# placeforyiming/DistanceTransform-DepthCompletion

Hardware: NVIDIA B200
Metric: DT+NN-fill frames/s @1216x352 (64-beam KITTI-shaped frames, batch 256 per GPU) (higher is better)
Workload: dtype u32 keys (integer chamfer) + f32 copy

## Files before the change

### distancetransform_depthcompletion_b200/csrc/dtfill.cu

```cuda
#include "dtfill.h"

#include <climits>
#include <cstdio>
#include <cstdlib>
#include <cstring>
#include <dlfcn.h>
#include <sched.h>

#include <atomic>
#include <condition_variable>
#include <functional>
#include <mutex>
#include <thread>
#include <string>
#include <vector>

#include "dtfill_kernels.cuh"

using namespace dtfill;

namespace {

thread_local std::string g_err;

// ... 214 lines not shown
                i = next_++;
                fn = fn_;
            }
            (*fn)(i);
            std::lock_guard<std::mutex> lk(mu_);
            if (++done_ == nparts_) cv_done_.notify_all();
        }
    }
    void loop() {
        for (;;) {
            {
                std::unique_lock<std::mutex> lk(mu_);
                cv_.wait(lk, [this] { return stop_ || next_ < nparts_; });
                if (stop_) return;
            }
            work();
        }
    }
    std::vector<std::thread> th_;
    std::mutex mu_;
    std::condition_variable cv_, cv_done_;
    bool stop_ = false;
    const std::function<void(size_t)>* fn_ = nullptr;
    size_t nparts_ = 0, next_ = 0, done_ = 0;
};

struct PinBuf {
    void* p = nullptr;
    size_t cap = 0;
};

struct Lane {
    static const int MAX_SUB = 16;
    Buf srcbits, wprefix, rowcell, rowsrc, rowval, counts, dlist, scratch, tasks, sky, skykeys;
    Buf ev_partial, ev_per_frame, ev_totals;
    bool ev_dirty = false;
    cudaStream_t sub[MAX_SUB] = {};
    cudaEvent_t fork_ev = nullptr, join_ev[MAX_SUB] = {};
    cudaStream_t side[MAX_SUB] = {};
    cudaEvent_t side_fork[MAX_SUB] = {}, side_join[MAX_SUB] = {};
    cudaStream_t pipe = nullptr;
    cudaStream_t pipe_front = nullptr;
    cudaEvent_t front_done = nullptr;
    cudaEvent_t done = nullptr;
    bool pending = false;
    int last_launches = 0;
    int last_B = 0;
};

struct dtfill_ctx {
    int device = 0;
    cudaStream_t own_stream = nullptr;
    cudaStream_t stream = nullptr;
    int sm_count = 148;
    static const int MAX_LANES = 4;
    Lane lanes[MAX_LANES];
    int ncalls = 0;
    int last_lane = 0;
    static const int STATUS_RING = 64;
    int* status_ring = nullptr;
    int* status_init = nullptr;
    bool slot_dirty[STATUS_RING] = {};
    cudaEvent_t slot_done[STATUS_RING] = {};
    int sticky_bad = INT_MAX;
    static const int STATUS_STRIDE = 64;
    int* status_dev = nullptr;
    bool slot_rearm[STATUS_RING] = {};
// ... 161 lines not shown
    if (is_src(ordered_to_float(lo))) return ordered_to_float(lo);
    while (hi - lo > 1) {
        const uint32_t mid = lo + (hi - lo) / 2;
        if (is_src(ordered_to_float(mid))) hi = mid; else lo = mid;
    }
    return ordered_to_float(hi);
}

int enqueue_range(dtfill_t* h, Lane* L, cudaStream_t s, cudaStream_t s_front, const Plan& plan, int b0, int nb, int Btot, const void* in, int H, int W,
                  float src_thr, float val_thr, float* out_depth, float* out_dt, int32_t* out_lbl, uint8_t* out_mask,
                  int32_t* out_counts, int scratch_units_per_frame, int sub_index, int* launches) {
    const int WW = (W + 31) / 32;
    const size_t rows0 = (size_t)b0 * H, npx0 = rows0 * W;
    const size_t rows = (size_t)nb * H;
    FrameParams fp;
    fp.B = nb; fp.H = H; fp.W = W; fp.WW = WW;
    fp.in_H = h->in_u16 ? h->in_H : H;
    fp.in_crop = h->in_u16 ? h->in_crop : 0;
    fp.src_thr = src_thr; fp.val_thr = val_thr;
    fp.src_cut = source_cut(src_thr);
    fp.init_dist = H + W + 8;
    fp.force_wide = plan.ppl == 0;
    fp.scratch_units_per_frame = scratch_units_per_frame;
    fp.wide_ppl = plan.ppl ? plan.ppl : 1;
    fp.narrow_ppl = (h->tiles2d && plan.ppl) ? plan.narrow : 0;
    fp.frame0 = b0;
    fp.sky_min = h->sky_min >= 0 ? h->sky_min : 8;
    fp.sky_split = (h->sky_split && !h->cur_pipelined && !h->profiling && h->tiles2d && plan.ppl && plan.narrow &&
                    h->narrow_main && fp.sky_min > 0 && W <= SKY_MAX_W && (long)Btot * H * W <= 28000000L) ? 1 : 0;
    fp.max_col_tiles = h->max_col_tiles;
    fp.mul_dist = 1u << (32 - DSH);
    fp.four = 4u;
    fp.one = 1u;
#ifdef DTFILL_TRACE
    fp.trace = h->trace_dev ? h->trace_dev + (size_t)(h->ncalls % dtfill_ctx::TRACE_CALLS) * 16 : nullptr;
#endif
    {
        int cap = h->band_cap;
        if (cap < 0) {
            const long beff = h->pipeline_depth > 1 ? (9L * Btot + 3) / 4 : Btot;
            const long per_frame = ((long)h->sm_count * 28 + beff - 1) / beff;
            if (per_frame <= 1) cap = 0;
            else {
                const long band_rows = (5L * H / 2) / per_frame;
                cap = (int)(2 * band_rows + 42);
                const int floor_cap = Btot <= 8 ? 80 : 96;
                if (cap < floor_cap) cap = floor_cap;
            }
        }
        fp.band_cap = plan.ppl ? cap : 0;
    }
    Workspace ws;
    ws.srcbits = (uint32_t*)L->srcbits.p + rows0 * WW;
    ws.wprefix = (uint16_t*)L->wprefix.p + rows0 * WW;
    ws.rowcell = (uint8_t*)L->rowcell.p + rows0 * WW;
    ws.rowsrc = (uint32_t*)L->rowsrc.p + rows0;
    ws.rowval = (uint32_t*)L->rowval.p + rows0;
    ws.counts = (int32_t*)L->counts.p + 2 * (size_t)b0;
    ws.dlist = (float*)L->dlist.p + npx0;
    ws.scratch = (uint32_t*)L->scratch.p + (size_t)b0 * scratch_units_per_frame * 32;
    ws.tasks = (Task*)L->tasks.p + (size_t)b0 * MAXT;
    ws.status = h->cur_status;
    ws.sky = (int*)L->sky.p + b0;
    ws.skykeys = (uint32_t*)L->skykeys.p + (size_t)b0 * 2 * W;
    float* olid = h->lidar_dev ? h->lidar_dev + npx0 : nullptr;
    float* od = out_depth + npx0;
    float* odt = out_dt ? out_dt + npx0 : nullptr;
    int32_t* ol = out_lbl ? out_lbl + npx0 : nullptr;
    uint8_t* om = out_mask ? out_mask + npx0 : nullptr;
    int32_t* oc = out_counts ? out_counts + 2 * (size_t)b0 : nullptr;

    if (h->profiling) CU(cudaEventRecord(h->ev[0], s));
    if (!(h->debug_skip & 1)) {
        const int k1_threads = 64;
        const int wpb = k1_threads / 32;
        long want = ((long)rows + wpb - 1) / wpb;
        int grid = (int)(want < 1 ? 1 : want);
        if (!h->in_u16) {
            const float* in_s = (const float*)in + npx0;
            if ((W & 15) == 0) k1_mask_rows_v16<float, true><<<grid, k1_threads, 0, s_front>>>(in_s, fp, ws, om, nullptr);
            else if ((W & 3) == 0) k1_mask_rows_v16<float, false><<<grid, k1_threads, 0, s_front>>>(in_s, fp, ws, om, nullptr);
            else k1_mask_rows<float><<<grid, k1_threads, 0, s_front>>>(in_s, fp, ws, om, nullptr);
        } else {
            const uint16_t* in_s = (const uint16_t*)in + (size_t)b0 * h->in_H * W;
            if ((W & 15) == 0) k1_mask_rows_v16<uint16_t, true><<<grid, k1_threads, 0, s_front>>>(in_s, fp, ws, om, olid);
            else if ((W & 7) == 0) k1_mask_rows_v16<uint16_t, false><<<grid, k1_threads, 0, s_front>>>(in_s, fp, ws, om, olid);
            else k1_mask_rows<uint16_t><<<grid, k1_threads, 0, s_front>>>(in_s, fp, ws, om, olid);
        }
        ++*launches;
        if (s_front != s) {
            CU(cudaEventRecord(L->front_done, s_front));
            CU(cudaStreamWaitEvent(s, L->front_done, 0));
        }
    }
    if (h->profiling) CU(cudaEventRecord(h->ev[1], s));
    if (!(h->debug_skip & 2)) {
        k1b_scan_compact<<<nb, K1B_THREADS, 0, s>>>(fp, ws, oc);
// ... 60 lines not shown
    if (h->profiling) CU(cudaEventRecord(h->ev[5], s));
    return 0;
}

int enqueue(dtfill_t* h, const void* in, int B, int H, int W, float src_thr, float val_thr, float* out_depth,
            float* out_dt, int32_t* out_lbl, uint8_t* out_mask, int32_t* out_counts, const HostIO* hio = nullptr,
            bool force_strict = false) {
    if (!h || !in || !out_depth) return fail(DTFILL_E_ARG, "dtfill_run: NULL handle, input or out_depth");
    if (B <= 0 || H <= 0 || W <= 0) return fail(DTFILL_E_ARG, "dtfill_run: B, H, W must be positive");
    if ((long)H + W >= 60000 || (long)H * W >= (1l << 31) || W > 28000)
        return fail(DTFILL_E_ARG, "dtfill_run: frame size not supported (H + W < 60000, W <= 28000)");
    CU(cudaSetDevice(h->device));
    const bool pipelined = h->pipeline_depth > 1 && !h->profiling && !hio && !force_strict;
    Lane* L = &h->lanes[pipelined ? (h->ncalls % h->pipeline_depth) : 0];
    h->cur_pipelined = pipelined;
    const Plan plan = make_plan(H, W);
    const int WW = (W + 31) / 32;
    const size_t rows = (size_t)B * H;
    const size_t npx = rows * W;

    int rc;
    if ((rc = ensure(h, L->srcbits, rows * WW * 4))) return rc;
    if ((rc = ensure(h, L->wprefix, rows * WW * 2))) return rc;
    if ((rc = ensure(h, L->rowcell, rows * WW))) return rc;
    if ((rc = ensure(h, L->rowsrc, rows * 4))) return rc;
    if ((rc = ensure(h, L->rowval, rows * 4))) return rc;
    if ((rc = ensure(h, L->counts, (size_t)B * 8))) return rc;
    if ((rc = ensure(h, L->dlist, npx * 4))) return rc;
    const int scratch_units_per_frame = plan.ppl ? 3 * H * plan.ppl : (int)(((size_t)H * W + 31) / 32);
    if ((rc = ensure(h, L->scratch, (size_t)B * scratch_units_per_frame * 128))) return rc;
    if ((rc = ensure(h, L->tasks, (size_t)B * MAXT * sizeof(Task)))) return rc;
    if ((rc = ensure(h, L->sky, (size_t)B * 4))) return rc;
    if ((rc = ensure(h, L->skykeys, (size_t)B * 2 * W * 4))) return rc;
    {
        const size_t smem = (size_t)3 * (W + 4) * sizeof(uint64_t);
        if (smem > 227 * 1024) return fail(DTFILL_E_ARG, "dtfill_run: frame too wide for the wide path");
        if (smem > 48 * 1024 && smem > h->wide_smem_configured) {
            CU(cudaFuncSetAttribute(k2_chamfer_wide, cudaFuncAttributeMaxDynamicSharedMemorySize, (int)smem));
            h->wide_smem_configured = smem;
        }
    }

    cudaStream_t s = h->stream, s_front = h->stream;
    if (pipelined) {
        CU(cudaEventRecord(h->pipe_fork, h->stream));
        s = L->pipe;
        if (h->prio_split) {
            s_front = L->pipe_front;
            CU(cudaStreamWaitEvent(s_front, h->pipe_fork, 0));
            if (L->pending) CU(cudaStreamWaitEvent(s_front, L->done, 0));
        } else {
            s_front = s;
            CU(cudaStreamWaitEvent(s, h->pipe_fork, 0));
        }
    } else {
        for (Lane& o : h->lanes)
            if (o.pending) { CU(cudaStreamWaitEvent(h->stream, o.done, 0)); o.pending = false; }
    }
    int launches = 0;
    const int slot = h->ncalls % dtfill_ctx::STATUS_RING;
    if (h->slot_dirty[slot]) {
        CU(cudaEventSynchronize(h->slot_done[slot]));
        if (h->status_ring[2 * slot] < h->sticky_bad) h->sticky_bad = h->status_ring[2 * slot];
        if (h->status_ring[2 * slot] != INT_MAX || h->status_ring[2 * slot + 1] != 0) h->slot_rearm[slot] = true;
        h->slot_dirty[slot] = false;
    }
// ... 214 lines not shown
        for (int i = 0; i < Lane::MAX_SUB; ++i) {
            CU(cudaStreamCreateWithFlags(&L.sub[i], cudaStreamNonBlocking));
            CU(cudaEventCreateWithFlags(&L.join_ev[i], cudaEventDisableTiming));
            CU(cudaStreamCreateWithPriority(&L.side[i], cudaStreamNonBlocking, prio_hi));
            CU(cudaEventCreateWithFlags(&L.side_fork[i], cudaEventDisableTiming));
            CU(cudaEventCreateWithFlags(&L.side_join[i], cudaEventDisableTiming));
        }
    }
    if (const char* e = getenv("DTFILL_PRIO_SPLIT")) h->prio_split = atoi(e) != 0;
    if (const char* e = getenv("DTFILL_TILES2D")) h->tiles2d = atoi(e) != 0;
    if (const char* e = getenv("DTFILL_SUBBATCHES")) h->nsub = atoi(e);
    if (const char* e = getenv("DTFILL_MAX_COL_TILES")) h->max_col_tiles = atoi(e);
    if (const char* e = getenv("DTFILL_SKY_MIN")) h->sky_min = atoi(e) < -1 ? -1 : atoi(e);
    if (const char* e = getenv("DTFILL_BAND_CAP")) h->band_cap = atoi(e);
    if (const char* e = getenv("DTFILL_NARROW_MAIN")) h->narrow_main = atoi(e) != 0;
    if (const char* e = getenv("DTFILL_SKY_SPLIT")) h->sky_split = atoi(e) != 0;
    if (const char* e = getenv("DTFILL_STAGE_THREADS")) h->stage_threads = atoi(e);
    if (const char* e = getenv("DTFILL_SPARSE_UPLOAD")) h->sparse_upload = atoi(e) != 0;
    if (const char* e = getenv("DTFILL_METRICS_EXACT")) h->metrics_exact = atoi(e) != 0;
    if (const char* e = getenv("DTFILL_PIPELINE_DEPTH")) {
        const int d = atoi(e);
        h->pipeline_depth = d < 1 ? 1 : (d > dtfill_ctx::MAX_LANES ? dtfill_ctx::MAX_LANES : d);
    }
    *out_handle = h;
    return 0;
}

void dtfill_destroy(dtfill_t* h) {
    if (!h) return;
    cudaSetDevice(h->device);
    cudaDeviceSynchronize();
    for (Lane& L : h->lanes) {
        Buf* lb[] = {&L.srcbits, &L.wprefix, &L.rowcell, &L.rowsrc, &L.rowval, &L.counts, &L.dlist,
                     &L.scratch, &L.tasks, &L.sky, &L.skykeys, &L.ev_partial, &L.ev_per_frame, &L.ev_totals};
        for (Buf* b : lb)
            if (b->p) cudaFree(b->p);
        if (L.fork_ev) cudaEventDestroy(L.fork_ev);
        if (L.done) cudaEventDestroy(L.done);
        if (L.pipe) cudaStreamDestroy(L.pipe);
        if (L.pipe_front) cudaStreamDestroy(L.pipe_front);
        if (L.front_done) cudaEventDestroy(L.front_done);
        for (int i = 0; i < Lane::MAX_SUB; ++i) {
            if (L.join_ev[i]) cudaEventDestroy(L.join_ev[i]);
            if (L.sub[i]) cudaStreamDestroy(L.sub[i]);
            if (L.side_fork[i]) cudaEventDestroy(L.side_fork[i]);
            if (L.side_join[i]) cudaEventDestroy(L.side_join[i]);
            if (L.side[i]) cudaStreamDestroy(L.side[i]);
        }
    }
    Buf* bufs[] = {&h->in_dev, &h->depth_dev, &h->dt_dev, &h->lbl_dev, &h->mask_dev, &h->counts_out_dev, &h->lidar_out_dev,
                   &h->gt_dev, &h->partial, &h->per_frame, &h->sums, &h->edt_rows, &h->edt_stack, &h->sparse_dev,
                   &h->mx_terms, &h->mx_counts, &h->mx_leaf_start, &h->mx_leaf_sum};
    for (Buf* b : bufs)
        if (b->p) cudaFree(b->p);
    for (void* q : h->retired) cudaFree(q);
    if (h->counts_host) cudaFreeHost(h->counts_host);
    delete h->pool_in;
    delete h->pool_out;
    for (PinBuf* b : {&h->pin_in, &h->pin_depth, &h->pin_dt, &h->pin_lbl, &h->pin_mask, &h->pin_lidar, &h->pin_sparse})
        if (b->p) cudaFreeHost(b->p);
    if (h->status_ring) cudaFreeHost(h->status_ring);
    if (h->status_dev) cudaFree(h->status_dev);
    if (h->status_stream) cudaStreamDestroy(h->status_stream);
    if (h->status_fork) cudaEventDestroy(h->status_fork);
    for (auto& e : h->slot_done)
        if (e) cudaEventDestroy(e);
    for (auto& e : h->ev)
// ... 738 lines not shown
```

### distancetransform_depthcompletion_b200/csrc/dtfill_common.cuh

```cuda
#pragma once
#include <cuda_runtime.h>
#include <stdint.h>

namespace dtfill {


constexpr int DSH = 21;
constexpr int OSH = 17;
constexpr uint32_t LMASK = (1u << OSH) - 1u;
constexpr uint32_t ORDCLR = ~(15u << OSH);
constexpr uint32_t MAX_FAST_LABEL = LMASK;
constexpr float UNREACHED_DT = 65533.0f;

__host__ __device__ constexpr uint32_t KC(int cost, int order) {
    return (uint32_t(cost) << DSH) | (uint32_t(order) << OSH);
}

enum TaskKind : int { TASK_CHAMFER = 0, TASK_NOSRC = 1, TASK_WIDE = 2, TASK_SKIP = 3, TASK_NARROW = 4 };

struct __align__(16) Task {
    int frame;
    int lo, hi;
    int r0, r1;
    int kind;
    int scratch_off;
    int fstart;
    int clo;
    int c0, c1;
    int sky;
};

constexpr int MAXT = 32;
constexpr int CELL_H = 4;
constexpr int CELL_W = 8;
constexpr int SKY_MAX_W = 1216;
constexpr int MAX_CELLS = 15360;

struct FrameParams {
    int B, H, W, WW;
    int in_H, in_crop;
    float src_thr, val_thr;
    float src_cut;
    int init_dist;
    int force_wide;
    int band_cap;
    int scratch_units_per_frame;
    int wide_ppl;
    int narrow_ppl;
    int max_col_tiles;
    int sky_min;
    int sky_split;
    int frame0;
    uint32_t mul_dist;
    uint32_t four;
    uint32_t one;
#ifdef DTFILL_TRACE
    unsigned long long* trace;
#endif
};

struct Workspace {
    uint32_t* srcbits;
    uint16_t* wprefix;
    uint8_t* rowcell;
    uint32_t* rowsrc;
    uint32_t* rowval;
    int32_t* counts;
    float* dlist;
    uint32_t* scratch;
    Task* tasks;
    int* sky;
    uint32_t* skykeys;
    int* status;
};

__device__ __forceinline__ float ld_stream(const float* p) {
    float v;
    asm volatile("ld.global.nc.L1::no_allocate.f32 %0, [%1];" : "=f"(v) : "l"(p));
    return v;
}
__device__ __forceinline__ void st_stream_u32(void* p, uint32_t v) {
    asm volatile("st.global.cs.u32 [%0], %1;" ::"l"(p), "r"(v));
}
__device__ __forceinline__ void st_stream_v4(void* p, uint32_t a, uint32_t b, uint32_t c, uint32_t d) {
    asm volatile("st.global.cs.v4.u32 [%0], {%1, %2, %3, %4};" ::"l"(p), "r"(a), "r"(b), "r"(c), "r"(d));
}
__device__ __forceinline__ float4 ld_stream_v4(const float* p) {
    float4 v;
    asm volatile("ld.global.nc.v4.f32 {%0, %1, %2, %3}, [%4];"
                 : "=f"(v.x), "=f"(v.y), "=f"(v.z), "=f"(v.w) : "l"(p));
    return v;
}
__device__ __forceinline__ uint4 ld_stream_v4u(const void* p) {
    uint4 v;
    asm volatile("ld.global.nc.v4.u32 {%0, %1, %2, %3}, [%4];" : "=r"(v.x), "=r"(v.y), "=r"(v.z), "=r"(v.w) : "l"(p));
    return v;
}
__device__ __forceinline__ float u16_depth(uint32_t v16) { return __uint_as_float(0x47000000u | v16) - 32768.0f; }
__device__ __forceinline__ float load_px_stream(const float* p) { return ld_stream(p); }
__device__ __forceinline__ float load_px_stream(const uint16_t* p) { return u16_depth(__ldg(p)); }

template <typename T> struct In16;
template <> struct In16<float> {
    float4 q[4];
    __device__ __forceinline__ void load(const float* p, int col, int W) {
// ... 80 lines not shown
```

### distancetransform_depthcompletion_b200/csrc/dtfill_k1b_plan.cuh

```cuda
#pragma once
#include "dtfill_common.cuh"

namespace dtfill {

constexpr int K1B_THREADS = 512;

__device__ __forceinline__ uint32_t block_exclusive_scan(uint32_t v, uint32_t* smem , uint32_t& total)
{
    constexpr int NW = K1B_THREADS / 32;
    const int lane = threadIdx.x & 31, wid = threadIdx.x >> 5;
    uint32_t inc = v;
#pragma unroll
    for (int d = 1; d < 32; d <<= 1) {
        const uint32_t o = __shfl_up_sync(0xffffffffu, inc, d);
        if (lane >= d) inc += o;
    }
    if (lane == 31) smem[wid] = inc;
    __syncthreads();
    if (threadIdx.x == 0) {
        uint32_t run = 0;
        for (int i = 0; i < NW; ++i) { const uint32_t t = smem[i]; smem[i] = run; run += t; }
        smem[NW] = run;
    }
    __syncthreads();
// ... 200 lines not shown
#pragma unroll
                for (int t = 0; t < 2; ++t) {
                    const uint32_t cin = __shfl_down_sync(0xffffffffu, e[t], 1);
                    d[t] = lane == 31 ? 120000u : cin;
                    mx[t] = 0;
#pragma unroll
                    for (int k = 7; k >= 0; --k)
                        if (k < chunk) { d[t] = min(d[t] + CELL_W, v[t][k]); if (xa + k < nw) mx[t] = max(mx[t], d[t]); }
                }
#pragma unroll
                for (int s_ = 16; s_ > 0; s_ >>= 1) {
#pragma unroll
                    for (int t = 0; t < 2; ++t) mx[t] = max(mx[t], __shfl_xor_sync(0xffffffffu, mx[t], s_));
                }
#pragma unroll
                for (int t = 0; t < 2; ++t) {
                    const int cy = cy0 + 8 * t;
                    if (lane == 0 && cy < nh) cellU[cy] = (int)min(mx[t], 60000u) + (CELL_H - 1) + (CELL_W - 1);
                }
            }
        } else {
            for (int cy = c0row + pw * 32 + lane; cy < nh; cy += 256) {
                uint32_t d = 60000;
                for (int cx = 0; cx < nw; ++cx) { d = min(d + CELL_W, (uint32_t)cellD[cy * nw + cx]); cellD[cy * nw + cx] = (uint16_t)min(d, 60000u); }
                d = 60000;
                uint32_t mx = 0;
                for (int cx = nw - 1; cx >= 0; --cx) { d = min(d + CELL_W, (uint32_t)cellD[cy * nw + cx]); mx = max(mx, min(d, 60000u)); }
                cellU[cy] = (int)mx + (CELL_H - 1) + (CELL_W - 1);
            }
        }
        planner_sync();
    }
    dbg_mark(4);

    if (ptid == 0) {
        ws.counts[2 * b] = (int)nsrc;
        ws.counts[2 * b + 1] = (int)nval;
        if (out_counts) { out_counts[2 * b] = (int)nsrc; out_counts[2 * b + 1] = (int)nval; }
        if (nval == 0 || nsrc > nval) atomicMin(&ws.status[0], b + fp.frame0);
        if (kind == TASK_WIDE) atomicAdd(&ws.status[1], 1);

        int nt = 0;
        Task* t = st;
        int* cost = scost;
        auto blank = [&](int knd) {
            Task q;
            q.frame = b; q.lo = 0; q.hi = H; q.r0 = 0; q.r1 = H; q.kind = knd; q.scratch_off = 0; q.fstart = 0;
            q.clo = 0; q.c0 = 0; q.c1 = W; q.sky = -2;
            return q;
        };
        int S = S0;
        if (plan) {
            const int nwid = fp.narrow_ppl * 32;
            int cy = S / CELL_H, scr = 0;
            bool ok = true;
            while (cy < nh && ok) {
                const int r0 = cy * CELL_H;
                int lo = 1 << 30, hi = 0, prev = 0, end = cy, best_lo = 0, best_hi = 0, umax = 0, best_u = 0;
                const bool base_band = fp.sky_split && S > 0 && r0 == S;
                for (int c = cy; c < nh; ++c) {
                    lo = min(lo, c * CELL_H - cellU[c]);
                    hi = max(hi, min(H, (c + 1) * CELL_H) + cellU[c]);
                    umax = max(umax, cellU[c]);
                    const int L = max(S, lo), Hh = min(H, hi);
                    const int cst = (Hh - L) + (Hh - r0);
                    const bool take = c == cy || (!base_band && (nt >= MAXT - 4 || cst <= fp.band_cap || cst - prev <= CELL_H ||
// ... 90 lines not shown
```

### distancetransform_depthcompletion_b200/csrc/dtfill_k2_chamfer.cuh

```cuda
#pragma once
#include "dtfill_common.cuh"

namespace dtfill {

template <int PPL>
struct Row {
    uint32_t v[PPL];
    uint32_t l1, l2;
    uint32_t r0, r1;
};

template <int PPL>
__device__ __forceinline__ uint32_t at(const Row<PPL>& r, int idx) {
    return idx == -2 ? r.l2 : idx == -1 ? r.l1 : idx == PPL ? r.r0 : idx == PPL + 1 ? r.r1 : r.v[idx < 0 ? 0 : (idx >= PPL ? PPL - 1 : idx)];
}

template <int PPL>
__device__ __forceinline__ void fill_row(Row<PPL>& r, uint32_t k) {
#pragma unroll
    for (int i = 0; i < PPL; ++i) r.v[i] = k;
    r.l1 = r.l2 = r.r0 = r.r1 = k;
}

template <int PPL>
// ... 57 lines not shown
}
__device__ __forceinline__ void st_scratch_v4_hint(void* p, uint32_t a, uint32_t b, uint32_t c, uint32_t d, uint64_t pol) {
    asm volatile("st.global.L2::cache_hint.v4.u32 [%0], {%1, %2, %3, %4}, %5;" ::"l"(p), "r"(a), "r"(b), "r"(c), "r"(d), "l"(pol) : "memory");
}
__device__ __forceinline__ void cp_async16_hint(uint32_t smem_addr, const void* gptr, uint64_t pol) {
    asm volatile("cp.async.cg.shared.global.L2::cache_hint [%0], [%1], 16, %2;" ::"r"(smem_addr), "l"(gptr), "l"(pol) : "memory");
}
__device__ __forceinline__ void l2_discard_128(const void* p) {
    asm volatile("discard.global.L2 [%0], 128;" ::"l"(p) : "memory");
}
__device__ __forceinline__ void mbar_init(uint32_t mbar, uint32_t count) {
    asm volatile("mbarrier.init.shared::cta.b64 [%0], %1;" ::"r"(mbar), "r"(count) : "memory");
    asm volatile("fence.mbarrier_init.release.cluster;" ::: "memory");
}
__device__ __forceinline__ void bulk_row_to_smem(uint32_t smem_dst, const void* gsrc, uint32_t bytes, uint32_t mbar) {
    asm volatile("mbarrier.arrive.expect_tx.shared::cta.b64 _, [%0], %1;" ::"r"(mbar), "r"(bytes) : "memory");
    asm volatile("cp.async.bulk.shared::cluster.global.mbarrier::complete_tx::bytes [%0], [%1], %2, [%3];"
                 ::"r"(smem_dst), "l"(gsrc), "r"(bytes), "r"(mbar) : "memory");
}
__device__ __forceinline__ void mbar_wait(uint32_t mbar, uint32_t parity) {
    uint32_t done = 0;
    while (!done)
        asm volatile("{\n\t.reg .pred p;\n\tmbarrier.try_wait.parity.shared::cta.b64 p, [%1], %2;\n\tselp.u32 %0, 1, 0, p;\n\t}"
                     : "=r"(done) : "r"(mbar), "r"(parity) : "memory");
}
__device__ __forceinline__ void cp_async_commit() { asm volatile("cp.async.commit_group;" ::: "memory"); }
template <int N>
__device__ __forceinline__ void cp_async_wait() { asm volatile("cp.async.wait_group %0;" ::"n"(N) : "memory"); }

__device__ __forceinline__ float key_dist_f32(uint32_t key, uint32_t mul_dist) {
    uint32_t t;
    asm("mad.hi.u32 %0, %1, %2, %3;" : "=r"(t) : "r"(key), "r"(mul_dist), "r"(0x4B000000u));
    return __uint_as_float(t) - 8388608.0f;
}

struct RowBits {
    uint32_t a, b, c, pre, base;
};

template <int PPL>
__device__ __forceinline__ RowBits fetch_row_bits(const uint32_t* __restrict__ bits_f, const uint16_t* __restrict__ pre_f,
                                                  const uint32_t* __restrict__ rowbase, int WW, int x0, int y)
{
    RowBits r;
    const int w = x0 >> 5;
    const uint32_t* br = bits_f + (long)y * WW;
    r.a = w < WW ? br[w] : 0u;
    r.b = w + 1 < WW ? br[w + 1] : 0u;
    r.c = (PPL > 33 && w + 2 < WW) ? br[w + 2] : 0u;
    r.pre = w < WW ? (uint32_t)pre_f[(long)y * WW + w] : 0u;
    r.base = rowbase[y];
    return r;
}

template <int PPL>
struct LaneBits { typedef uint64_t type; };
template <> struct LaneBits<10> { typedef uint32_t type; };
template <> struct LaneBits<20> { typedef uint32_t type; };

template <int PPL>
__device__ __forceinline__ void decode_row_bits(const RowBits& r, int x0, typename LaneBits<PPL>::type& bits,
                                                uint32_t& rank)
{
    const int sh = x0 & 31;
    if (sizeof(typename LaneBits<PPL>::type) == 4) {
        bits = __funnelshift_r(r.a, r.b, sh) & ((1u << (PPL & 31)) - 1u);
    } else {
        uint64_t lo = ((uint64_t)r.b << 32) | r.a;
        lo >>= sh;
        if (PPL > 33 && sh) lo |= (uint64_t)r.c << (64 - sh);
        bits = (typename LaneBits<PPL>::type)(lo & ((PPL >= 64) ? ~0ull : ((1ull << PPL) - 1ull)));
    }
    rank = r.base + r.pre + __popc(r.a & ((1u << sh) - 1u)) + 1u;
}


#ifndef DTFILL_STENCIL
#define DTFILL_STENCIL 1
#endif
#ifndef DTFILL_SPLITSCAN
#define DTFILL_SPLITSCAN 1
#endif
#ifndef DTFILL_FAKE_SCRATCH_DIV
#define DTFILL_FAKE_SCRATCH_DIV 1
#endif
#ifndef DTFILL_L2POLICY
#define DTFILL_L2POLICY 0
#endif
#ifndef DTFILL_K2_TMA
#define DTFILL_K2_TMA 1
#endif
#ifndef DTFILL_FLUSH_LATE
#define DTFILL_FLUSH_LATE 0
#endif
#ifndef DTFILL_K2_SMEMROW
#define DTFILL_K2_SMEMROW 0
#endif
#ifndef DTFILL_K2_WARPS
#define DTFILL_K2_WARPS (DTFILL_K2_SMEMROW ? 28 : 20)
#endif

template <int PPL>
__device__ __forceinline__ void load_row_smem(Row<PPL>& r, const uint32_t* row, int lane, uint32_t init_key) {
    const uint4* p = reinterpret_cast<const uint4*>(row + lane * PPL);
#pragma unroll
    for (int j = 0; j < PPL / 4; ++j) {
        const uint4 q = p[j];
        r.v[4 * j] = q.x; r.v[4 * j + 1] = q.y; r.v[4 * j + 2] = q.z; r.v[4 * j + 3] = q.w;
    }
    const uint32_t a = row[lane == 0 ? 0 : lane * PPL - 1], c = row[lane == 31 ? 0 : lane * PPL + PPL];
    r.l1 = lane == 0 ? init_key : a;
    r.r0 = lane == 31 ? init_key : c;
    r.l2 = r.r1 = init_key;
}
template <int PPL>
__device__ __forceinline__ void store_row_smem(uint32_t* row, const Row<PPL>& r, int lane) {
    uint4* p = reinterpret_cast<uint4*>(row + lane * PPL);
#pragma unroll
    for (int j = 0; j < PPL / 4; ++j) p[j] = make_uint4(r.v[4 * j], r.v[4 * j + 1], r.v[4 * j + 2], r.v[4 * j + 3]);
}

template <int PPL>
__device__ __forceinline__ uint32_t stencil_fwd(const Row<PPL>& A , const Row<PPL>& Bq , int i, uint32_t one)
{
    const uint32_t b0 = at(Bq, i - 1), b1 = at(Bq, i + 1);
    const uint32_t a0 = at(A, i - 2), a1 = at(A, i - 1), a2 = at(A, i), a3 = at(A, i + 1), a4 = at(A, i + 2);
#if DTFILL_STENCIL == 0
    uint32_t m = b0 * one + KC(3, 0);
    m = __viaddmin_u32(b1, KC(3, 2), m);
    m = __viaddmin_u32(a0, KC(3, 4), m);
    m = __viaddmin_u32(a1, KC(2, 6), m);
    m = __viaddmin_u32(a2, KC(1, 8), m);
// ... 65 lines not shown
    __shared__ __align__(16) uint2 fwdbuf[16 * PPL];
#if DTFILL_K2_TMA
    __shared__ __align__(8) uint64_t fwdbar;
#endif

    const Task task = ws.tasks[blockIdx.x];
    if (task.kind != my_kind && !(task.kind == TASK_NOSRC && my_kind == TASK_CHAMFER)) return;
    DTFILL_TRACE_SCOPE(fp, 2);
    const int lane = threadIdx.x;
    const int H = fp.H, W = fp.W, WW = fp.WW;
    const int b = task.frame;
    const long fpx = (long)b * H * W;

    if (task.kind == TASK_NOSRC) {
        const int nval = ws.counts[2 * b + 1];
        const float last = ws.dlist[fpx + (nval > 0 ? nval - 1 : 0)];
        for (long i = (long)task.r0 * W + lane; i < (long)task.r1 * W; i += 32) {
            out_depth[fpx + i] = last;
            if (out_dt) out_dt[fpx + i] = UNREACHED_DT;
            if (WANT_LBL) out_lbl[fpx + i] = 0;
        }
        return;
    }

    const int x0 = task.clo + lane * PPL;
    const int xl = lane * PPL;
    const uint32_t init_key = (uint32_t)fp.init_dist << DSH;
    const uint32_t clamp_dist = 2047u - PPL - 1u;
    const uint32_t* bits_f = ws.srcbits + (long)b * H * WW;
    const uint16_t* pre_f = ws.wprefix + (long)b * H * WW;
    const uint32_t* rowbase = ws.rowsrc + (long)b * H;
    constexpr int VW = (PPL % 4 == 0) ? 4 : 2;
    uint2* scr = reinterpret_cast<uint2*>(ws.scratch) + (long)task.scratch_off * 16;

#if DTFILL_L2POLICY
    const uint64_t pol_keep = l2_policy_evict_last(), pol_drop = l2_policy_evict_first();
#endif
    Row<PPL> ra, rb;
    fill_row(ra, init_key);
    fill_row(rb, init_key);

    RowBits nextbits = fetch_row_bits<PPL>(bits_f, pre_f, rowbase, WW, x0, task.fstart);
    auto fwd_step = [&](const Row<PPL>& A , Row<PPL>& Bq , int y) {
        typename LaneBits<PPL>::type bits; uint32_t rank;
        decode_row_bits<PPL>(nextbits, x0, bits, rank);
        nextbits = fetch_row_bits<PPL>(bits_f, pre_f, rowbase, WW, x0, min(y + 1, task.hi - 1));
        if (lane < 2 && y + 4 < task.hi) {
            asm volatile("prefetch.global.L2 [%0];" ::"l"(bits_f + (long)(y + 4) * WW + (x0 >> 5) + lane * 32));
            asm volatile("prefetch.global.L2 [%0];" ::"l"(pre_f + (long)(y + 4) * WW + (x0 >> 5) + lane * 32));
        }
        uint32_t c[PPL];
#pragma unroll
        for (int i = 0; i < PPL; ++i) c[i] = stencil_fwd<PPL>(A, Bq, i, fp.one);
        if (__any_sync(0xffffffffu, bits != 0)) {
#pragma unroll
            for (int i = 0; i < PPL; ++i) {
                const bool s = (bits & ((typename LaneBits<PPL>::type)1 << i)) != 0;
                c[i] = s ? rank : c[i];
                rank += s ? 1u : 0u;
            }
        }
#if DTFILL_SPLITSCAN
        constexpr int HF = PPL / 2;
        uint32_t u = c[0] & ORDCLR, u2 = c[HF] & ORDCLR;
        c[0] = u; c[HF] = u2;
#pragma unroll
        for (int i = 1; i < PPL - HF; ++i) {
            if (i < HF) { u = __viaddmin_u32(u, KC(1, 14), c[i]) & ORDCLR; c[i] = u; }
            u2 = __viaddmin_u32(u2, KC(1, 14), c[HF + i]) & ORDCLR; c[HF + i] = u2;
        }
        const uint32_t e = __viaddmin_u32(u | (1u << OSH), uint32_t(PPL - HF) << DSH, u2) & ORDCLR;
        const uint32_t cin = lane_carry<PPL, +1>(e, lane, clamp_dist);
        const uint32_t cin2 = __viaddmin_u32(cin, uint32_t(HF) << DSH, u) | (1u << OSH);
#pragma unroll
        for (int i = 0; i < PPL; ++i) {
            uint32_t t = i < HF ? __viaddmin_u32(cin, uint32_t(i + 1) << DSH, c[i])
                                : __viaddmin_u32(cin2, uint32_t(i - HF + 1) << DSH, c[i]);
            if (PAD && x0 + i >= W) t = init_key;
            Bq.v[i] = t;
        }
#else
        uint32_t u = c[0] & ORDCLR;
        c[0] = u;
#pragma unroll
        for (int i = 1; i < PPL; ++i) {
            u = __viaddmin_u32(u, KC(1, 14), c[i]) & ORDCLR;
            c[i] = u;
        }
        const uint32_t cin = lane_carry<PPL, +1>(u, lane, clamp_dist);
#pragma unroll
        for (int i = 0; i < PPL; ++i) {
            uint32_t t = __viaddmin_u32(cin, uint32_t(i + 1) << DSH, c[i]);
            if (PAD && x0 + i >= W) t = init_key;
            Bq.v[i] = t;
        }
#endif
        refresh_halo(Bq, lane, init_key);
        if (y >= task.r0) {
            char* dst = reinterpret_cast<char*>(scr) + (long)(y - task.lo) * (128 * PPL) + lane * (4 * VW);
#pragma unroll
            for (int j = 0; j < PPL / VW / DTFILL_FAKE_SCRATCH_DIV; ++j) {
#if DTFILL_L2POLICY
                if (VW == 4) st_scratch_v4_hint(dst + j * 512, Bq.v[4 * j], Bq.v[4 * j + 1], Bq.v[4 * j + 2], Bq.v[4 * j + 3], pol_keep);
#else
                if (VW == 4) st_scratch_v4(dst + j * 512, Bq.v[4 * j], Bq.v[4 * j + 1], Bq.v[4 * j + 2], Bq.v[4 * j + 3]);
#endif
                else st_scratch_v2(dst + j * 256, Bq.v[2 * j], Bq.v[2 * j + 1]);
            }
        }
    };

    if (SB) {
        store_row_smem<PPL>(stage_ring, ra, lane);
        store_row_smem<PPL>(stage_ring + 32 * PPL, ra, lane);
        __syncwarp();
#pragma unroll 1
        for (int y = task.fstart; y < task.hi; ++y) {
            uint32_t* slot = stage_ring + (y & 1) * (32 * PPL);
            load_row_smem<PPL>(rb, slot, lane, init_key);
            fwd_step(ra, rb, y);
            __syncwarp();
            store_row_smem<PPL>(slot, rb, lane);
            ra = rb;
        }
        __syncwarp();
    } else {
#pragma unroll 1
    for (int y = task.fstart; y < task.hi; ++y) {
        fwd_step(ra, rb, y);
        const Row<PPL> t = ra; ra = rb; rb = t;
    }
// ... 13 lines not shown
    uint32_t okmask = 0;
#pragma unroll
    for (int j = 0; j < NJ; ++j) {
        const int lc = (j * 32 + lane) * 4, col = task.clo + lc;
        if (lc < 32 * PPL && col >= task.c0 && col < task.c1) okmask |= 1u << j;
    }
    const long colbase = fpx + task.clo + lane * 4;
    const uint4* sread0 = reinterpret_cast<const uint4*>(&stage[lane * 4]);
    uint2* swrite0 = reinterpret_cast<uint2*>(&stage[xl]);
    const uint32_t fwdbuf_lane = (uint32_t)__cvta_generic_to_shared(fwdbuf) + lane * (4 * VW);

#if DTFILL_K2_TMA
    constexpr bool TMA_ROWS = (VW == 4) && DTFILL_FAKE_SCRATCH_DIV == 1;
#else
    constexpr bool TMA_ROWS = false;
#endif
#if DTFILL_K2_TMA
    const uint32_t fwdbar_a = (uint32_t)__cvta_generic_to_shared(&fwdbar);
    const uint32_t fwdbuf_a = (uint32_t)__cvta_generic_to_shared(fwdbuf);
    if (TMA_ROWS) {
        if (lane == 0) mbar_init(fwdbar_a, 1);
        asm volatile("fence.proxy.async;" ::: "memory");
        __syncwarp();
    }
    uint32_t fwd_phase = 0;
    bool fwd_inflight = false;
#endif
    auto issue_fwd_row = [&](int y) {
        const bool have = y >= task.fstart && y >= task.lo;
#if DTFILL_K2_TMA
        if (TMA_ROWS) {
            fwd_inflight = have;
            if (have && lane == 0)
                bulk_row_to_smem(fwdbuf_a, reinterpret_cast<const char*>(scr) + (long)(y - task.lo) * (128 * PPL), 128 * PPL, fwdbar_a);
            return;
        }
#endif
        if (have) {
            const char* src = reinterpret_cast<const char*>(scr) + (long)(y - task.lo) * (128 * PPL) + lane * (4 * VW);
#pragma unroll
            for (int j = 0; j < PPL / VW / DTFILL_FAKE_SCRATCH_DIV; ++j) {
#if DTFILL_L2POLICY
                if (VW == 4) cp_async16_hint(fwdbuf_lane + j * 512, src + j * 512, pol_drop);
#else
                if (VW == 4) cp_async16_l2only(fwdbuf_lane + j * 512, src + j * 512);
#endif
                else cp_async8(fwdbuf_lane + j * 256, src + j * 256);
            }
        }
        cp_async_commit();
    };
    auto wait_fwd_row = [&]() {
#if DTFILL_K2_TMA
        if (TMA_ROWS) {
            if (fwd_inflight) { mbar_wait(fwdbar_a, fwd_phase); fwd_phase ^= 1u; }
            return;
        }
#endif
        cp_async_wait<0>();
    };
    uint32_t g[NJ * 4];
    auto flush_depth_row = [&](int y) {
        float* pd = out_depth + colbase + (long)y * W;
#pragma unroll
        for (int j = 0; j < NJ; ++j)
            if ((okmask >> j) & 1u) st_stream_v4(pd + j * 128, g[4 * j], g[4 * j + 1], g[4 * j + 2], g[4 * j + 3]);
    };

    issue_fwd_row(task.hi - 1);

    auto bwd_step = [&](const Row<PPL>& A , Row<PPL>& Bq , int y) {
        if (lane < PPL / DTFILL_FAKE_SCRATCH_DIV && y - 3 >= task.fstart)
            asm volatile("prefetch.global.L2 [%0];" ::"l"(reinterpret_cast<const char*>(scr) +
                                                          (long)(y - 3 - task.lo) * (128 * PPL) + lane * 128));
#if DTFILL_FLUSH_LATE == 0
        if (VEC && y + 1 >= task.r0 && y + 1 < task.r1) flush_depth_row(y + 1);
#endif
        wait_fwd_row();
#if DTFILL_L2POLICY >= 2
        if (VW == 4 && lane < PPL && y >= task.fstart && y >= task.lo)
            l2_discard_128(reinterpret_cast<const char*>(scr) + (long)(y - task.lo) * (128 * PPL) + lane * 128);
#endif
        uint32_t c[PPL];
        if (y >= task.fstart) {
#pragma unroll
            for (int j = 0; j < PPL / VW; ++j) {
                if (DTFILL_FAKE_SCRATCH_DIV > 1 && j >= PPL / VW / DTFILL_FAKE_SCRATCH_DIV) {
                    for (int e = 0; e < VW; ++e) c[VW * j + e] = init_key;
                } else if (VW == 4) {
                    const uint4 f = reinterpret_cast<const uint4*>(fwdbuf)[j * 32 + lane];
                    c[4 * j] = f.x; c[4 * j + 1] = f.y; c[4 * j + 2] = f.z; c[4 * j + 3] = f.w;
                } else {
                    const uint2 f = fwdbuf[j * 32 + lane];
                    c[2 * j] = f.x; c[2 * j + 1] = f.y;
                }
            }
        } else {
#pragma unroll
            for (int i = 0; i < PPL; ++i) c[i] = init_key;
        }
#pragma unroll
        for (int i = 0; i < PPL; ++i) c[i] = stencil_bwd<PPL>(c[i], A, Bq, i, fp.one) & ORDCLR;
#if DTFILL_K2_TMA
        if (TMA_ROWS) __syncwarp();
#endif
        issue_fwd_row(y - 1);
#if DTFILL_FLUSH_LATE == 1
        if (VEC && y + 1 >= task.r0 && y + 1 < task.r1) flush_depth_row(y + 1);
#endif
#if DTFILL_SPLITSCAN
        constexpr int HF = PPL / 2;
        uint32_t u = c[PPL - 1], u2 = c[HF - 1];
#pragma unroll
        for (int i = 1; i < PPL - HF; ++i) {
            u = __viaddmin_u32(u, KC(1, 1), c[PPL - 1 - i]) & ORDCLR; c[PPL - 1 - i] = u;
            if (i < HF) { u2 = __viaddmin_u32(u2, KC(1, 1), c[HF - 1 - i]) & ORDCLR; c[HF - 1 - i] = u2; }
        }
// ... 113 lines not shown
```

Before: 614,300.

## Compress forward-pass scratch rows to 16-bit keys when cell bounds allow

New measurement: 585,400, median of 6. -4.7%, worse.

```diff
diff --git a/distancetransform_depthcompletion_b200/csrc/dtfill.cu b/distancetransform_depthcompletion_b200/csrc/dtfill.cu
--- a/distancetransform_depthcompletion_b200/csrc/dtfill.cu
+++ b/distancetransform_depthcompletion_b200/csrc/dtfill.cu
@@ -270,7 +270,7 @@
 
 struct Lane {
     static const int MAX_SUB = 16;
-    Buf srcbits, wprefix, rowcell, rowsrc, rowval, counts, dlist, scratch, tasks, sky, skykeys;
+    Buf srcbits, wprefix, rowcell, rowsrc, rowval, counts, dlist, scratch, tasks, sky, skykeys, cellu;
     Buf ev_partial, ev_per_frame, ev_totals;
     bool ev_dirty = false;
     cudaStream_t sub[MAX_SUB] = {};
@@ -498,6 +498,13 @@
     fp.mul_dist = 1u << (32 - DSH);
     fp.four = 4u;
     fp.one = 1u;
+    fp.m16 = 1u << 16;
+    for (int f = 0; f < 2; ++f) {
+        const uint32_t db = 4 + f, ob = 16 - db;
+        fp.f16[f].m32 = 1u << (32 - ob); fp.f16[f].mo = 1u << ob; fp.f16[f].m16o = 1u << (16 + ob);
+        fp.f16[f].sat2 = ((1u << db) - 1u) * 0x10001u;
+        fp.f16[f].md = 1u << db; fp.f16[f].kd = (1u << DSH) - (1u << ob);
+    }
 #ifdef DTFILL_TRACE
     fp.trace = h->trace_dev ? h->trace_dev + (size_t)(h->ncalls % dtfill_ctx::TRACE_CALLS) * 16 : nullptr;
 #endif
@@ -529,6 +536,7 @@
     ws.status = h->cur_status;
     ws.sky = (int*)L->sky.p + b0;
     ws.skykeys = (uint32_t*)L->skykeys.p + (size_t)b0 * 2 * W;
+    ws.cellu = (int*)L->cellu.p + (size_t)b0 * ((H + CELL_H - 1) / CELL_H);
     float* olid = h->lidar_dev ? h->lidar_dev + npx0 : nullptr;
     float* od = out_depth + npx0;
     float* odt = out_dt ? out_dt + npx0 : nullptr;
@@ -655,6 +663,7 @@
     if ((rc = ensure(h, L->tasks, (size_t)B * MAXT * sizeof(Task)))) return rc;
     if ((rc = ensure(h, L->sky, (size_t)B * 4))) return rc;
     if ((rc = ensure(h, L->skykeys, (size_t)B * 2 * W * 4))) return rc;
+    if ((rc = ensure(h, L->cellu, (size_t)B * ((H + CELL_H - 1) / CELL_H) * 4))) return rc;
     {
         const size_t smem = (size_t)3 * (W + 4) * sizeof(uint64_t);
         if (smem > 227 * 1024) return fail(DTFILL_E_ARG, "dtfill_run: frame too wide for the wide path");
@@ -935,7 +944,7 @@
     cudaDeviceSynchronize();
     for (Lane& L : h->lanes) {
         Buf* lb[] = {&L.srcbits, &L.wprefix, &L.rowcell, &L.rowsrc, &L.rowval, &L.counts, &L.dlist,
-                     &L.scratch, &L.tasks, &L.sky, &L.skykeys, &L.ev_partial, &L.ev_per_frame, &L.ev_totals};
+                     &L.scratch, &L.tasks, &L.sky, &L.skykeys, &L.cellu, &L.ev_partial, &L.ev_per_frame, &L.ev_totals};
         for (Buf* b : lb)
             if (b->p) cudaFree(b->p);
         if (L.fork_ev) cudaEventDestroy(L.fork_ev);
diff --git a/distancetransform_depthcompletion_b200/csrc/dtfill_common.cuh b/distancetransform_depthcompletion_b200/csrc/dtfill_common.cuh
--- a/distancetransform_depthcompletion_b200/csrc/dtfill_common.cuh
+++ b/distancetransform_depthcompletion_b200/csrc/dtfill_common.cuh
@@ -35,6 +35,12 @@
 constexpr int CELL_W = 8;
 constexpr int SKY_MAX_W = 1216;
 constexpr int MAX_CELLS = 15360;
+constexpr int CELLU_NONE = 60000;
+
+struct Fwd16Format {
+    uint32_t m32, mo, m16o, sat2;
+    uint32_t md, kd;
+};
 
 struct FrameParams {
     int B, H, W, WW;
@@ -54,6 +60,8 @@
     uint32_t mul_dist;
     uint32_t four;
     uint32_t one;
+    uint32_t m16;
+    Fwd16Format f16[2];
 #ifdef DTFILL_TRACE
     unsigned long long* trace;
 #endif
@@ -71,6 +79,7 @@
     Task* tasks;
     int* sky;
     uint32_t* skykeys;
+    int* cellu;
     int* status;
 };
 
diff --git a/distancetransform_depthcompletion_b200/csrc/dtfill_k1b_plan.cuh b/distancetransform_depthcompletion_b200/csrc/dtfill_k1b_plan.cuh
--- a/distancetransform_depthcompletion_b200/csrc/dtfill_k1b_plan.cuh
+++ b/distancetransform_depthcompletion_b200/csrc/dtfill_k1b_plan.cuh
@@ -256,6 +256,11 @@
         planner_sync();
     }
     dbg_mark(4);
+
+    if (pw > 0) {
+        int* cu = ws.cellu + (long)b * nh;
+        for (int cy = ptid - 32; cy < nh; cy += 256 - 32) cu[cy] = (plan && cy >= c0row) ? cellU[cy] : CELLU_NONE;
+    }
 
     if (ptid == 0) {
         ws.counts[2 * b] = (int)nsrc;
diff --git a/distancetransform_depthcompletion_b200/csrc/dtfill_k2_chamfer.cuh b/distancetransform_depthcompletion_b200/csrc/dtfill_k2_chamfer.cuh
--- a/distancetransform_depthcompletion_b200/csrc/dtfill_k2_chamfer.cuh
+++ b/distancetransform_depthcompletion_b200/csrc/dtfill_k2_chamfer.cuh
@@ -113,6 +113,31 @@
     uint32_t t;
     asm("mad.hi.u32 %0, %1, %2, %3;" : "=r"(t) : "r"(key), "r"(mul_dist), "r"(0x4B000000u));
     return __uint_as_float(t) - 8388608.0f;
+}
+
+__device__ __forceinline__ uint32_t fwd16_pack(uint32_t k0, uint32_t k1, uint32_t nb, const Fwd16Format& F, const FrameParams& fp) {
+    uint32_t a0, a1, off, d0, d1, w;
+    asm("mad.lo.u32 %0, %1, %2, %3;" : "=r"(a0) : "r"(k0), "r"(F.m32), "r"(nb));
+    asm("mad.lo.u32 %0, %1, %2, %3;" : "=r"(a1) : "r"(k1), "r"(F.m32), "r"(nb));
+    asm("mad.hi.u32 %0, %1, %2, %3;" : "=r"(off) : "r"(a0), "r"(F.mo), "r"(0u));
+    asm("mad.hi.u32 %0, %1, %2, %3;" : "=r"(off) : "r"(a1), "r"(F.m16o), "r"(off));
+    asm("mad.hi.u32 %0, %1, %2, %3;" : "=r"(d0) : "r"(k0), "r"(fp.mul_dist), "r"(0u));
+    asm("mad.hi.u32 %0, %1, %2, %3;" : "=r"(d1) : "r"(k1), "r"(fp.mul_dist), "r"(0u));
+    asm("mad.lo.u32 %0, %1, %2, %3;" : "=r"(d0) : "r"(d1), "r"(fp.m16), "r"(d0));
+    d0 = __vminu2(d0, F.sat2);
+    asm("mad.lo.u32 %0, %1, %2, %3;" : "=r"(w) : "r"(d0), "r"(F.mo), "r"(off));
+    return w;
+}
+__device__ __forceinline__ void fwd16_unpack(uint32_t w, uint32_t base1, const Fwd16Format& F, const FrameParams& fp,
+                                             uint32_t& k0, uint32_t& k1) {
+    uint32_t x, e0, e1, d0, d1;
+    asm("mad.lo.u32 %0, %1, %2, %3;" : "=r"(x) : "r"(w), "r"(fp.m16), "r"(0u));
+    asm("mad.hi.u32 %0, %1, %2, %3;" : "=r"(e0) : "r"(x), "r"(fp.m16), "r"(base1));
+    asm("mad.hi.u32 %0, %1, %2, %3;" : "=r"(d0) : "r"(x), "r"(F.md), "r"(0u));
+    asm("mad.hi.u32 %0, %1, %2, %3;" : "=r"(e1) : "r"(w), "r"(fp.m16), "r"(base1));
+    asm("mad.hi.u32 %0, %1, %2, %3;" : "=r"(d1) : "r"(w), "r"(F.md), "r"(0u));
+    asm("mad.lo.u32 %0, %1, %2, %3;" : "=r"(k0) : "r"(d0), "r"(F.kd), "r"(e0));
+    asm("mad.lo.u32 %0, %1, %2, %3;" : "=r"(k1) : "r"(d1), "r"(F.kd), "r"(e1));
 }
 
 struct RowBits {
@@ -175,10 +200,10 @@
 #define DTFILL_FLUSH_LATE 0
 #endif
 #ifndef DTFILL_K2_SMEMROW
-#define DTFILL_K2_SMEMROW 0
+#define DTFILL_K2_SMEMROW 1
 #endif
 #ifndef DTFILL_K2_WARPS
-#define DTFILL_K2_WARPS (DTFILL_K2_SMEMROW ? 28 : 20)
+#define DTFILL_K2_WARPS 20
 #endif
 
 template <int PPL>
@@ -310,6 +335,37 @@
     const uint32_t* rowbase = ws.rowsrc + (long)b * H;
     constexpr int VW = (PPL % 4 == 0) ? 4 : 2;
     uint2* scr = reinterpret_cast<uint2*>(ws.scratch) + (long)task.scratch_off * 16;
+    char* const scr_c = reinterpret_cast<char*>(scr);
+
+    constexpr bool FWD16 = PPL == 20 && DTFILL_K2_TMA && DTFILL_FAKE_SCRATCH_DIV == 1 && DTFILL_L2POLICY < 2;
+    constexpr int ROW16 = 16 + 64 * PPL;
+    bool use16 = false;
+    if (FWD16) {
+        const int ys = max(task.r0, task.fstart);
+        const int* cu = ws.cellu + (long)b * ((H + CELL_H - 1) / CELL_H);
+        int umax = 0;
+        for (int c = task.r0 / CELL_H + lane; c * CELL_H < task.r1; c += 32)
+            if (min(c * CELL_H + CELL_H, task.r1) > ys) umax = max(umax, cu[c]);
+        if (__reduce_max_sync(0xffffffffu, umax) <= 30) {
+            const uint32_t nsrc = (uint32_t)ws.counts[2 * b];
+            bool fits = true;
+            for (int y = ys + lane; y < task.hi; y += 32) {
+                int T = 0;
+                for (int c = task.r0 / CELL_H; c * CELL_H < task.r1; ++c) {
+                    const int yn = min(max(y, c * CELL_H), min(c * CELL_H + CELL_H, task.r1) - 1);
+                    T = max(T, cu[c] - abs(y - yn));
+                }
+                const uint32_t first = rowbase[max(task.lo, y - T)];
+                const uint32_t span = (y + 1 < H ? rowbase[y + 1] : nsrc) - first;
+                const uint32_t db = (T <= 14 && span <= 4096u) ? 4u : (T <= 30 && span <= 2048u) ? 5u : 0u;
+                fits = fits && db != 0u;
+                *reinterpret_cast<uint4*>(scr_c + (long)(y - task.lo) * ROW16) = make_uint4(first + 1u, db, 0u, 0u);
+            }
+            use16 = __all_sync(0xffffffffu, fits);
+            __syncwarp();
+        }
+    }
+    const int row_bytes = use16 ? ROW16 : 128 * PPL;
 
 #if DTFILL_L2POLICY
     const uint64_t pol_keep = l2_policy_evict_last(), pol_drop = l2_policy_evict_first();
@@ -322,6 +378,8 @@
     auto fwd_step = [&](const Row<PPL>& A , Row<PPL>& Bq , int y) {
         typename LaneBits<PPL>::type bits; uint32_t rank;
         decode_row_bits<PPL>(nextbits, x0, bits, rank);
+        uint2 hdr = make_uint2(0u, 0u);
+        if (FWD16 && use16 && y >= task.r0) hdr = *reinterpret_cast<const uint2*>(scr_c + (long)(y - task.lo) * ROW16);
         nextbits = fetch_row_bits<PPL>(bits_f, pre_f, rowbase, WW, x0, min(y + 1, task.hi - 1));
         if (lane < 2 && y + 4 < task.hi) {
             asm volatile("prefetch.global.L2 [%0];" ::"l"(bits_f + (long)(y + 4) * WW + (x0 >> 5) + lane * 32));
@@ -374,7 +432,20 @@
         }
 #endif
         refresh_halo(Bq, lane, init_key);
-        if (y >= task.r0) {
+        if (FWD16 && use16 && y >= task.r0) {
+            uint32_t w[PPL / 2];
+            auto pack = [&](const Fwd16Format& F) {
+                const uint32_t nb = 0u - hdr.x * F.m32;
+#pragma unroll
+                for (int m = 0; m < PPL / 2; ++m) w[m] = fwd16_pack(Bq.v[2 * m], Bq.v[2 * m + 1], nb, F, fp);
+            };
+            if (hdr.y == 4u) pack(fp.f16[0]); else pack(fp.f16[1]);
+            char* dst = scr_c + (long)(y - task.lo) * ROW16 + 16;
+#pragma unroll
+            for (int j = 0; j < PPL / 8; ++j)
+                st_scratch_v4(dst + j * 512 + lane * 16, w[4 * j], w[4 * j + 1], w[4 * j + 2], w[4 * j + 3]);
+            if (PPL % 8) st_scratch_v2(dst + (PPL / 8) * 512 + lane * 8, w[PPL / 2 - 2], w[PPL / 2 - 1]);
+        } else if (y >= task.r0) {
             char* dst = reinterpret_cast<char*>(scr) + (long)(y - task.lo) * (128 * PPL) + lane * (4 * VW);
 #pragma unroll
             for (int j = 0; j < PPL / VW / DTFILL_FAKE_SCRATCH_DIV; ++j) {
@@ -454,7 +525,7 @@
         if (TMA_ROWS) {
             fwd_inflight = have;
             if (have && lane == 0)
-                bulk_row_to_smem(fwdbuf_a, reinterpret_cast<const char*>(scr) + (long)(y - task.lo) * (128 * PPL), 128 * PPL, fwdbar_a);
+                bulk_row_to_smem(fwdbuf_a, scr_c + (long)(y - task.lo) * row_bytes, row_bytes, fwdbar_a);
             return;
         }
 #endif
@@ -492,9 +563,8 @@
     issue_fwd_row(task.hi - 1);
 
     auto bwd_step = [&](const Row<PPL>& A , Row<PPL>& Bq , int y) {
-        if (lane < PPL / DTFILL_FAKE_SCRATCH_DIV && y - 3 >= task.fstart)
-            asm volatile("prefetch.global.L2 [%0];" ::"l"(reinterpret_cast<const char*>(scr) +
-                                                          (long)(y - 3 - task.lo) * (128 * PPL) + lane * 128));
+        if (lane * 128 < row_bytes / DTFILL_FAKE_SCRATCH_DIV && y - 3 >= task.fstart)
+            asm volatile("prefetch.global.L2 [%0];" ::"l"(scr_c + (long)(y - 3 - task.lo) * row_bytes + lane * 128));
 #if DTFILL_FLUSH_LATE == 0
         if (VEC && y + 1 >= task.r0 && y + 1 < task.r1) flush_depth_row(y + 1);
 #endif
@@ -505,6 +575,32 @@
 #endif
         uint32_t c[PPL];
         if (y >= task.fstart) {
+          if (FWD16 && use16) {
+            const uint2 h = reinterpret_cast<const uint2*>(fwdbuf)[0];
+            const char* fb = reinterpret_cast<const char*>(fwdbuf) + 16;
+            uint32_t w[PPL / 2];
+#pragma unroll
+            for (int j = 0; j < PPL / 8; ++j) {
+                const uint4 q = reinterpret_cast<const uint4*>(fb + j * 512)[lane];
+                w[4 * j] = q.x; w[4 * j + 1] = q.y; w[4 * j + 2] = q.z; w[4 * j + 3] = q.w;
+            }
+            if (PPL % 8) {
+                const uint2 q = reinterpret_cast<const uint2*>(fb + (PPL / 8) * 512)[lane];
+                w[PPL / 2 - 2] = q.x; w[PPL / 2 - 1] = q.y;
+            }
+            __syncwarp();
+            auto unpack = [&](const Fwd16Format& F) {
+#pragma unroll
+                for (int j = 0; j < PPL / 4; ++j) {
+                    uint4 k;
+                    fwd16_unpack(w[2 * j], h.x, F, fp, k.x, k.y);
+                    fwd16_unpack(w[2 * j + 1], h.x, F, fp, k.z, k.w);
+                    reinterpret_cast<uint4*>(fwdbuf)[j * 32 + lane] = k;
+                }
+            };
+            if (h.y == 4u) unpack(fp.f16[0]); else unpack(fp.f16[1]);
+            __syncwarp();
+          }
 #pragma unroll
             for (int j = 0; j < PPL / VW; ++j) {
                 if (DTFILL_FAKE_SCRATCH_DIV > 1 && j >= PPL / VW / DTFILL_FAKE_SCRATCH_DIV) {
```
